# MrinalJain17/CT-image-segmentation

Hardware: AMD Instinct MI355X
Metric: CT volumes/sec training (512x512x48, bs=2/GPU) (higher is better)
Workload: dtype bf16; 1 GPU; 3D U-Net (MONAI UNet, channels 32-64-128-256, 2 res units) training step on 2x1x512x512x48 synthetic CT volumes per GPU (BASELINE.json configs[2]), CrossEntropy + Dice metric + Adam; global_batch=2, parallelism=dp1

## Files before the change

### ct-image-segmentation_amd/capstone_amd/_native.py

```python
import ctypes as C
import os

import torch

_HERE = os.path.dirname(os.path.abspath(__file__))
LIB_PATH = os.environ.get("CTSEG_LIB") or os.path.join(os.path.dirname(_HERE), "lib", "libctseg_hip.so")

F32, BF16, I16, U8, F16 = 0, 1, 2, 3, 4
MAX_TAPS, MAX_CLASSES = 27, 8
ABI_VERSION = 3
_TORCH_DT = {F32: torch.float32, BF16: torch.bfloat16, F16: torch.float16}
_EPC = {F32: 4, BF16: 8, F16: 8}
_SZ = {F32: 4, BF16: 2, F16: 2}
DT_OF_PRECISION = {"fp32": F32, "bf16": BF16, "fp16": F16}


def is16(dt):
    return dt in (BF16, F16)


def torch_dtype(dt):
    return _TORCH_DT[dt]


# ... 104 lines not shown
    "ctseg_instnorm_prelu_bwd_apply": (C.c_int, [_i32, _vp, _i32, _vp, _i32, _vp, _vp, _vp, _vp, _i32, _vp, _i32, _i32, _i64, _i32,
                                                 _vp, _i32, _vp, _vp]),
    "ctseg_instnorm_prelu_bwd_apply_colsum": (C.c_int, [_i32, _vp, _i32, _vp, _i32, _vp, _vp, _vp, _vp, _i32, _vp, _i32, _i32, _i64, _i32,
                                                        _vp, _i32, _vp, _vp, _i32, _vp, _vp]),
    "ctseg_colsum": (C.c_int, [_i32, _vp, _i32, _i64, _i32, _vp, _i32, _vp, _vp]),
    "ctseg_batchnorm_finalize": (C.c_int, [_vp, _i32, _i32, _i32, _i32, _i32, _f64, _f64, _f64, _vp, _vp, _vp, _vp, _vp, _vp, _vp, _vp]),
    "ctseg_batchnorm_eval_table": (C.c_int, [_vp, _vp, _vp, _vp, _i32, _f64, _vp, _vp]),
    "ctseg_scale_shift_prelu_fwd": (C.c_int, [_i32, _vp, _i32, _vp, _vp, _vp, _i32, _vp, _i32, _i32, _i64, _i32, _vp]),
    "ctseg_batchnorm_prelu_bwd_reduce": (C.c_int, [_i32, _vp, _i32, _vp, _i32, _vp, _vp, _vp, _vp, _vp, _i32, _i32, _i32, _i64, _i32,
                                                   _vp]),
    "ctseg_batchnorm_prelu_bwd_finalize": (C.c_int, [_vp, _i32, _i32, _i32, _i32, _f64, _vp, _vp, _vp, _vp, _vp]),
    "ctseg_batchnorm_prelu_bwd_apply": (C.c_int, [_i32, _vp, _i32, _vp, _i32, _vp, _vp, _vp, _vp, _vp, _vp, _i32, _vp, _i32, _i32,
                                                  _i64, _i32, _vp, _i32, _vp, _vp]),
    "ctseg_squash_masks": (C.c_int, [_vp, _i32, _i32, _i64, _vp, _vp, _vp, _vp]),
    "ctseg_squash_masks_present": (C.c_int, [_vp, _i32, _i32, _i64, _vp, _vp, _vp, _vp, _vp]),
    "ctseg_mixup_images": (C.c_int, [_vp, _vp, _i32, _i64, _f64, _vp, _vp]),
    "ctseg_seg_loss_pair": (C.c_int, [_vp, _i32, _vp, _vp, _i32, _i64, _i32, _vp, _i32, _vp, _i32, _vp, _vp, _vp, _i32, _i32, _vp]),
    "ctseg_seg_loss": (C.c_int, [_vp, _i32, _vp, _i32, _i64, _i32, _vp, _i32, _vp, _i32, _vp, _i32, _vp, _vp, _i32, _i32, _vp, _vp]),
    "ctseg_conv_logits_ce_slots": (C.c_int, [C.POINTER(ConvDesc), _i32]),
    "ctseg_conv_logits_ce": (C.c_int, [C.POINTER(ConvDesc), _vp, _i32, _vp, _vp, _i32, _vp, _i32, _vp, _i32, _i32, _vp, _vp]),
    "ctseg_dice_counts": (C.c_int, [_vp, _vp, _i32, _i64, _i32, _vp, _vp]),
    "ctseg_reduce_partials_f64": (C.c_int, [_vp, _i32, _i32, _i32, _vp, _vp]),
    "ctseg_loss_dice_summary": (C.c_int, [_vp, _i32, _i32, _vp, _i32, _vp, _vp]),
    "ctseg_adam_step": (C.c_int, [_vp, _vp, _vp, _vp, _i64, _f64, _f64, _f64, _f64, _i32, _f32, _vp]),
    "ctseg_scale_inplace": (C.c_int, [_vp, _i32, _i64, _vp, _f32, _vp]),
    "ctseg_cast": (C.c_int, [_vp, _i32, _vp, _i32, _i64, _vp]),
    "ctseg_nc_to_cl": (C.c_int, [_vp, _vp, _i32, _i32, _i32, _i64, _i32, _vp]),
    "ctseg_cl_to_nc": (C.c_int, [_vp, _i32, _vp, _i32, _i32, _i64, _i32, _vp]),
    "ctseg_resize3d_to_hwd": (C.c_int, [_vp, _i32, _vp] + [_i32] * 8 + [_f32, _f32, _vp, _vp, _vp, _vp, _vp]),
    "ctseg_window_gather": (C.c_int, [_vp] + [_i32] * 10 + [_f32, _vp, _i32, _i32, _vp]),
    "ctseg_window_gather_batch": (C.c_int, [_vp] + [_i32] * 4 + [_vp] + [_i32] * 4 + [_f32, _vp, _i32, _i32, _vp]),
    "ctseg_window_blend": (C.c_int, [_vp] + [_i32] * 8 + [_vp, _vp, _vp] + [_i32] * 4 + [_vp]),
    "ctseg_window_blend_batch": (C.c_int, [_vp] + [_i32] * 5 + [_vp, _i32, _vp, _vp, _vp] + [_i32] * 4 + [_vp, _vp]),
}
EXPORTS = tuple(_SIGS)
_lib = None


def lib():
    global _lib
    if _lib is None:
        if not os.path.exists(LIB_PATH):
            raise NativeError(f"{LIB_PATH} is missing: run `python -c 'import __graft_entry__ as g; g.build()'` "
                              "(or `make -C ct-image-segmentation_amd`). There is no CPU/eager fallback.")
        L = C.CDLL(LIB_PATH)
        for name, (res, args) in _SIGS.items():
            fn = getattr(L, name)
# ... 34 lines not shown
```

### ct-image-segmentation_amd/capstone_amd/engine.py

```python
import ctypes as C
import math
import os

import numpy as np
import torch

from . import _native as nat
from ._native import BF16, F32


def rup(a, b):
    return (a + b - 1) // b * b


class Act:
    __slots__ = ("t", "C", "c0", "dt", "pending_norm", "bst")

    def __init__(self, t, C, c0=0, dt=None):
        self.t, self.C, self.c0 = t, C, c0
        self.pending_norm = None
        self.bst = None
        self.dt = dt if dt is not None else {torch.float32: F32, torch.float16: nat.F16}.get(t.dtype, BF16)

    @property
# ... 135 lines not shown
    def g_ptr(self, p):
        return self.flat_g.data_ptr() + 4 * self.offsets[id(p)]

    def grad_view(self, p):
        o = self.offsets[id(p)]
        return self.flat_g[o:o + p.numel()].view(p.shape)

    def grad_views(self):
        if self._grad_views is None:
            self._grad_views = [self.grad_view(p) for p in self.params]
        return self._grad_views

    def version(self):
        return (self.generation, sum(p._version for p in self.params))

    def touch(self):
        self.generation += 1

    def ensure_adam_state(self):
        if self.adam_m is None:
            self.adam_m = torch.zeros_like(self.flat_g)
            self.adam_v = torch.zeros_like(self.flat_g)

    def adam_step(self, lr, betas=(0.9, 0.999), eps=1e-8, grad_scale=1.0):
        self.ensure_adam_state()
        self.step += 1
        nat.call("ctseg_adam_step", self.flat_p.data_ptr(), self.flat_g.data_ptr(), self.adam_m.data_ptr(),
                 self.adam_v.data_ptr(), self.n, lr, betas[0], betas[1], eps, self.step, grad_scale)
        self.touch()


class BufferStore:

    def __init__(self, norms, device):
        self.norms = list(norms)
        self.device = device
        self.offsets, off = {}, 0
        for i, m in enumerate(self.norms):
            self.offsets[id(m)] = (off, i)
            off += 2 * m.num_features
        self.flat = torch.zeros(max(off, 4), dtype=torch.float32, device=device)
        self.nbt = torch.zeros(max(len(self.norms), 1), dtype=torch.int64, device=device)
        self.copy_in()

    def _views(self, m):
        o, i = self.offsets[id(m)]
        C = m.num_features
        return self.flat[o:o + C], self.flat[o + C:o + 2 * C], self.nbt[i]

    def copy_in(self):
        with torch.no_grad():
            for m in self.norms:
# ... 323 lines not shown
                col0 += cout
        else:
            w, b, cout = self.parts[0]
            plan.emit("ctseg_conv_wgrad_reduce", ws.data_ptr(), nslabs, kpad_w, cn_pad, A, cg, self.T, 0, cn,
                      st.g_ptr(w), None)
            if b is not None and not bias_done:
                plan.emit_colsum(dy, st.g_ptr(b))


class NormStats:
    def __init__(self, plan, N, tiles, C, count):
        self.plan, self.N, self.tiles, self.C, self.count = plan, N, tiles, C, count
        self.ld = rup(C, 256 if C > 128 else nat.lib().ctseg_conv_tile_cols(C))
        self.partials = torch.zeros((N, tiles, 2, self.ld), dtype=torch.float32, device=plan.device)
        self.scratch = torch.zeros(N * 64 * 2 * self.ld + N, dtype=torch.float64, device=plan.device)

    def emit_finalize(self, col0, C, eps=1e-5):
        mr = torch.zeros((self.N, C, 2), dtype=torch.float32, device=self.plan.device)
        self.plan.emit("ctseg_instnorm_finalize", self.partials.data_ptr(), self.N, self.tiles, self.ld, col0, C,
                       float(self.count), float(eps), self.scratch.data_ptr(), mr.data_ptr(), keep=(self, mr))
        return mr


class Packer:
    def __init__(self, plan):
        self.plan = plan
        self.blocks = []
        self.descs = []
        self.total = 0
        self.bias_blocks, self.bias_total = [], 0
        self.first = (0, 0)
        self.buf = self.bias_buf = None
        self.idx = self.bias_idx = None
        self.n_idx = self.n_bidx = 0
        self.pack_blocks = self.pack_rows = None
        self.n_pack_blocks = self.n_pack_rows = 0
        self.n_first_rows = 0
        self.dirty = True
        self.version = None

    def add(self, layer, mode):
        dt = self.plan.dt
        bk = 128 // nat.elsize(dt)
        zero = self.plan.store.zero_index
        classes = layer.fwd_classes if mode == "fwd" else layer.dg_classes
        rows, gs = layer.rows_gather(mode)
        rows_pad = rup(rows, 256 if rows > 128 else 128)
        info = {"kpads": [], "w_offs": [], "base": self.total}
        for _, taps in classes:
            nt = len(taps)
            kpad = rup(nt * gs, bk)
            n_, t_, g_ = np.broadcast_arrays(np.arange(rows_pad)[:, None, None],
                                             np.array([t for t, _ in taps])[None, :, None],
                                             np.arange(gs)[None, None, :])
            src = np.where(n_ < rows, layer.src_index(mode, n_, g_, t_), zero)
            blk = np.full((rows_pad, kpad), zero, dtype=np.int64)
            blk[:, :nt * gs] = src.reshape(rows_pad, nt * gs)
            info["kpads"].append(kpad)
            info["w_offs"].append(self.total - info["base"])
            self.blocks.append((self.total, blk.reshape(-1)))
# ... 50 lines not shown
        self.dirty = True
        fits = all(sum((min(gh, d["gs"]) - gl) * d["T"] for (_, _, _, gl, gh, _, _) in d["parts"]) <= nat.PACK_LDS_FLOATS and
                   len(d["parts"]) <= 2 for d in self.descs)
        if self.descs and fits:
            arr = (nat.PackBlock * len(self.descs))()
            rows = []
            for b, d in enumerate(self.descs):
                B = arr[b]
                B.dst_off, B.kpad, B.gs, B.ntaps, B.T, B.nparts = d["dst_off"], d["kpad"], d["gs"], d["ntaps"], d["T"], len(d["parts"])
                for j, t in enumerate(d["taps"]):
                    B.tap[j] = t
                for k, (o, n_lo, n_hi, g_lo, g_hi, SN, SG) in enumerate(d["parts"]):
                    P = B.part[k]
                    P.o, P.n_lo, P.n_hi, P.g_lo, P.g_hi, P.SN, P.SG = o, n_lo, n_hi, g_lo, min(g_hi, d["gs"]), SN, SG
                rows += [(b, n) for n in range(d["rows"])]
            raw = torch.frombuffer(bytearray(bytes(arr)), dtype=torch.uint8).clone()
            self.pack_blocks = raw.to(dev)
            lo, hi = self.first
            head = [(b, n) for (b, n) in rows if lo <= self.descs[b]["dst_off"] < hi]
            rest = [(b, n) for (b, n) in rows if not (lo <= self.descs[b]["dst_off"] < hi)]
            self.n_first_rows = len(head)
            self.pack_rows = torch.tensor(head + rest, dtype=torch.int32).reshape(-1).to(dev)
            self.n_pack_blocks, self.n_pack_rows = len(self.descs), len(rows)

    def can_split(self):
        return self.pack_blocks is not None and self.n_first_rows > 0

    def stale(self):
        return self.dirty or self.plan.store.version() != self.version

    def refresh(self, force=False, part=None):
        st = self.plan.store
        ver = st.version()
        if not (force or self.dirty or ver != self.version):
            return
        if self.pack_blocks is not None:
            lo, hi = {None: (0, self.n_pack_rows), "first": (0, self.n_first_rows), "rest": (self.n_first_rows, self.n_pack_rows)}[part]
            if hi > lo:
                nat.call("ctseg_pack_weights", st.flat_p.data_ptr(), self.pack_blocks.data_ptr(), self.n_pack_blocks,
                         self.pack_rows.data_ptr() + 8 * lo, hi - lo, self.buf.data_ptr(), self.plan.dt)
        elif part != "rest":
            nat.call("ctseg_gather_cast", st.flat_p.data_ptr(), self.idx.data_ptr(), self.buf.data_ptr(), self.plan.dt, self.n_idx)
        if part != "rest":
            nat.call("ctseg_gather_cast", st.flat_p.data_ptr(), self.bias_idx.data_ptr(), self.bias_buf.data_ptr(), F32, self.n_bidx)
        if part != "first":
            self.dirty, self.version = False, ver
# ... 1 lines not shown
```

### ct-image-segmentation_amd/capstone_amd/plan.py

```python
import math
import os

import torch
import torch.nn as nn

from . import _native as nat
from ._native import BF16, F32
from .engine import Act, BufferStore, GemmLayer, NarrowUnsupported, Packer, ParamStore, plan_act, rup


def _is_seq(m):
    return isinstance(m, nn.Sequential) and not hasattr(m, "conv_only")


def _bwd_row_ranges(S, N, dt):
    P = max(1, min(1024, math.ceil(S / 512)))
    if nat.is16(dt):
        P = max(P, min(math.ceil(1024 / N), math.ceil(S / 32)))
    return P


def _parts(conv):
    return (conv.weight, conv.bias, conv.out_channels)

# ... 475 lines not shown
            return
        offs = [self.store.off(p) for p in params if p is not None]
        if self._pending_reduce:
            self._pending_ready.extend(offs)
            self._flush_reduces(only_if_chunk=True)
        else:
            self.ready_marks.append((len(self.bwd), offs))

    @staticmethod
    def run(prog, stream, lo=0, hi=None):
        for name, fn, args in prog[lo:hi]:
            rc = fn(*args, stream)
            if rc != 0:
                nat.check(rc, name)

    def load_input(self, x):
        N, X, Y, Z = self.shape
        cin = self.x.C
        xs = x.reshape(N, cin, X * Y * Z)
        if not xs.is_contiguous() or xs.dtype != torch.float32:
            xs = xs.contiguous().float()
        nat.call("ctseg_nc_to_cl", xs.data_ptr(), self.x.t.data_ptr(), self.dt, N, cin, X * Y * Z, cin)

    def repack_after_update(self):
        side = self.side_stream()
        if side is None:
            self.packer.dirty = True
            return
        main = torch.cuda.current_stream(self.device)
        side.wait_stream(main)
        with torch.cuda.stream(side):
            if self.packer.can_split():
                self.packer.refresh(force=True, part="first")
                self._repack_ev = side.record_event()
                self.packer.refresh(force=True, part="rest")
                self._repack_ev2 = side.record_event()
            else:
                self.packer.refresh(force=True)
                self._repack_ev = side.record_event()

    def head_ce_slots(self, n_classes):
        cache = self._head_ce
        if cache is None or cache[0] != n_classes:
            slots = 0
            name, _, args = self.fwd[-1]
            if name == "ctseg_conv_igemm" and not self.inference and args[0].out == self.logits.ptr():
                slots = nat.lib().ctseg_conv_logits_ce_slots(args[0], n_classes)
            cache = self._head_ce = (n_classes, max(slots, 0), args[0])
        return cache[1]

    def forward(self, x=None, skip_head=False):
        if x is not None:
            self.load_input(x)
        if self._repack_ev is not None:
            torch.cuda.current_stream(self.device).wait_event(self._repack_ev)
# ... 350 lines not shown
```

### ct-image-segmentation_amd/capstone_amd/segloss.py

```python
import contextlib
import math

import torch

from . import _native as nat
from ._native import BF16, F32

N_CLASSES = 10
CLASS_WEIGHT = (1e-10, 0.007, 0.3296, 0.0046, 0.2619, 0.3035, 0.0068, 0.0065, 0.0374, 0.0426)
SMOOTH = 1e-5
LOSS_NAMES = ("CrossEntropy", "WeightedCrossEntropy", "Focal", "Dice", "GeneralizedDice")


def cl_logits(t):
    if t.dtype != torch.float32 or not t.is_cuda or t.ndim < 3:
        return None
    perm = (0,) + tuple(range(2, t.ndim)) + (1,)
    v = t.permute(perm)
    st, sh = v.stride(), v.shape
    if st[-1] != 1:
        return None
    ld = st[-2] if v.ndim > 2 else sh[-1]
    exp = ld
    for d in range(v.ndim - 2, -1, -1):
# ... 52 lines not shown

    def set_labels_from_i64(self, target):
        t = target.reshape(self.B, self.S)
        self.labels = t.to(torch.uint8).contiguous()
        self.hist = torch.zeros((self.B, self.C), dtype=torch.int64, device=self.device)
        self.hist.scatter_add_(1, t.long(), torch.ones_like(t, dtype=torch.int64))

    def _pass(self, logits_ptr, ld, cw, do_stats, do_grad, coef=None, dl_ptr=None, g_ld=0, gdt=F32, pred=None, part=None):
        nat.call("ctseg_seg_loss", logits_ptr, ld, self.labels.data_ptr(), self.B, self.S, self.C, nat.ptr(cw),
                 int(do_stats), nat.ptr(part if part is not None else self.part), self.P, self.cnt.data_ptr(),
                 int(do_grad), nat.ptr(coef), dl_ptr, g_ld, gdt, nat.ptr(pred))

    def stats(self, logits_ptr, ld, weighted_too=False):
        self.cnt.zero_()
        self._pass(logits_ptr, ld, None, True, False)
        nat.call("ctseg_reduce_partials_f64", self.part.data_ptr(), self.B, self.P, self.R, self.red.data_ptr())
        if weighted_too:
            keep = self.cnt.clone()
            self._pass(logits_ptr, ld, self.cw, True, False)
            nat.call("ctseg_reduce_partials_f64", self.part.data_ptr(), self.B, self.P, self.R, self.red_w.data_ptr())
            self.cnt.copy_(keep)

    def prepare_fused_ce(self, weighted=False):
        self.cnt.zero_()
        w = self.cw.double() if weighted else torch.ones(self.C, dtype=torch.float64, device=self.device)
        denom = (self.hist.double() * w[None, :]).sum()
        self.coef.zero_()
        self.coef[:, 0] = (1.0 / denom).float()
        self._ce_ready = weighted

    def _take_ce_tables(self, weighted):
        if self._ce_ready is not weighted:
            self.prepare_fused_ce(weighted)
        self._ce_ready = None

    def fused_ce(self, logits_ptr, ld, dl_ptr, g_ld, gdt, weighted=False):
        self._take_ce_tables(weighted)
        self._pass(logits_ptr, ld, self.cw if weighted else None, 2, 2, self.coef, dl_ptr, g_ld, gdt)
        nat.call("ctseg_reduce_partials_f64", self.part.data_ptr(), self.B, self.P, self.R,
                 (self.red_w if weighted else self.red).data_ptr())

    def head_ce(self, desc, slots, dl_ptr, g_ld, weighted=False):
        self._take_ce_tables(weighted)
        part = self._part_head
        if part is None or part.shape[1] != slots:
            part = self._part_head = torch.zeros((self.B, slots, self.R), dtype=torch.float64, device=self.device)
        nat.call("ctseg_conv_logits_ce", desc, self.labels.data_ptr(), self.C, nat.ptr(self.cw if weighted else None),
                 self.coef.data_ptr(), self.coef.shape[1], dl_ptr, g_ld, part.data_ptr(), slots, self.R, self.cnt.data_ptr())
        nat.call("ctseg_reduce_partials_f64", part.data_ptr(), self.B, slots, self.R, (self.red_w if weighted else self.red).data_ptr())

    def ce_summary(self, weighted=False):
# ... 191 lines not shown
```

### ct-image-segmentation_amd/capstone_amd/volumetric/base_trainer.py

```python
from argparse import ArgumentParser
from typing import List

import torch
import torch.nn as nn

from .. import STRUCTURES, segloss
from .. import _native as nat
from ..models import UNet
from ..training.utils import _squash_predictions
from .losses import MultipleLossWrapper3D
from .metrics import DiceMetricWrapper3D
from .utils import _squash_masks_3D

try:
    import pytorch_lightning as pl
    _Base = pl.LightningModule
except Exception:
    pl = None

    class _HParams(dict):
        __getattr__ = dict.__getitem__

    class _Base(nn.Module):

# ... 271 lines not shown
            le.build_coef({n: 1.0 for n in names})
            le.grad(logits.ptr(), logits.ld, dl.ptr(), dl.ld, plan.dt)
        book = {}

        def bookkeeping():
            if ce_only:
                loss, dm, dpc = le.ce_summary(weighted=names[0] != "CrossEntropy")
                book["vals"], book["total"], book["dice"], book["packed"] = {names[0]: loss}, loss, (dm, dpc), le.last_summary
                return
            book["vals"] = vals
            book["total"] = torch.stack([vals[n] for n in names]).sum()
            book["dice"] = le.dice_metric()

        self._keep_dice_counts(le.cnt, "train")

        reducer = eng.reducer
        if reducer is not None:
            plan.backward(reducer.hooks(plan), before_join=bookkeeping)
            scale = reducer.finish()
        else:
            eng.warn_if_unattached()
            plan.backward(before_join=bookkeeping)
            scale = 1.0
        eng.store.adam_step(self.hparams.lr, betas, eps, grad_scale=scale)
        plan.repack_after_update()
        vals, total = book["vals"], book["total"]
        dice_mean, dice_per_class = book["dice"]
        if "packed" in book and pl is None:
            self.log_packed(book["packed"], [(f"{names[0]} Loss (train)", 0), ("Mean Dice Score (train)", 1),
                                             ("Dice per class (train)", slice(2, None))] +
                            [(f"{s_} Dice (train)", 2 + i) for i, s_ in enumerate(STRUCTURES)])
        else:
            for n in names:
                self.log(f"{n} Loss (train)", vals[n], on_step=False, on_epoch=True)
            self.log("Mean Dice Score (train)", dice_mean, on_step=False, on_epoch=True)
            if pl is None:
                self.log("Dice per class (train)", dice_per_class, on_step=False, on_epoch=True)
            else:
                for structure, score in zip(STRUCTURES, dice_per_class):
                    self.log(f"{structure} Dice (train)", score, on_step=False, on_epoch=True)
        return total

    def optimizer_state_dict(self, betas=(0.9, 0.999), eps=1e-8):
        st = self.unet.engine().store
        params = list(self.parameters())
        state = {}
        if st is not None and st.step > 0:
            for i, p in enumerate(params):
# ... 62 lines not shown
```

### ct-image-segmentation_amd/csrc/loss_metric.hip

```cpp
#include "loss_common.h"

namespace ctseg {

template <bool PRESENT>
__global__ __launch_bounds__(256) void squash_masks_kernel(const uint8_t* __restrict__ masks, int K, int64_t S,
                                                           uint8_t* __restrict__ labels, int64_t* __restrict__ labels_i64,
                                                           unsigned long long* __restrict__ hist, int* __restrict__ present) {
  __shared__ unsigned int s_h[32];
  __shared__ unsigned int s_pres;
  const int b = blockIdx.y;
  if (threadIdx.x < 32) s_h[threadIdx.x] = 0;
  if (PRESENT && threadIdx.x == 0) s_pres = 0u;
  unsigned int pres = 0u;
  __syncthreads();
  const uint8_t* mb = masks + (int64_t)b * K * S;
  int bg = 0;
  const bool vec = (S % 16 == 0) && (((uintptr_t)masks % 16) == 0) && (((uintptr_t)labels % 16) == 0);
  const int64_t nchunk = (S + 15) / 16;
  for (int64_t ch = blockIdx.x * (int64_t)blockDim.x + threadIdx.x; ch < nchunk; ch += (int64_t)gridDim.x * blockDim.x) {
    const int64_t v0 = ch * 16;
    int lab[16];
#pragma unroll
    for (int i = 0; i < 16; ++i) lab[i] = 0;
    if (vec) {
      for (int k = 0; k < K; ++k) {
        const u32x4 m = *reinterpret_cast<const u32x4*>(mb + (int64_t)k * S + v0);
        if constexpr (PRESENT) {
          unsigned int hit = 0u;
#pragma unroll
          for (int w = 0; w < 4; ++w) { const uint32_t z = m[w] ^ 0x01010101u; hit |= (z - 0x01010101u) & ~z & 0x80808080u; }
          if (hit) pres |= 1u << k;
        }
#pragma unroll
        for (int i = 0; i < 16; ++i) {
          const int val = (int)((m[i >> 2] >> (8 * (i & 3))) & 0xffu) * (k + 1);
          lab[i] = val > lab[i] ? val : lab[i];
        }
      }
      u32x4 o;
#pragma unroll
      for (int w = 0; w < 4; ++w)
        o[w] = (uint32_t)(lab[4 * w] & 0xff) | ((uint32_t)(lab[4 * w + 1] & 0xff) << 8) | ((uint32_t)(lab[4 * w + 2] & 0xff) << 16) |
               ((uint32_t)(lab[4 * w + 3] & 0xff) << 24);
      *reinterpret_cast<u32x4*>(labels + (int64_t)b * S + v0) = o;
    } else {
      for (int i = 0; i < 16; ++i) {
        if (v0 + i >= S) break;
        int l = 0;
        for (int k = 0; k < K; ++k) {
          const int mv = (int)mb[(int64_t)k * S + v0 + i];
          if (PRESENT && mv == 1) pres |= 1u << k;
          const int val = mv * (k + 1);
          l = val > l ? val : l;
        }
        lab[i] = l;
        labels[(int64_t)b * S + v0 + i] = (uint8_t)l;
      }
    }
    int nbg = 0;
#pragma unroll
    for (int i = 0; i < 16; ++i) {
      if (v0 + i < S) {
        if (labels_i64 != nullptr) labels_i64[(int64_t)b * S + v0 + i] = lab[i];
        if (lab[i] == 0) ++nbg;
        else if (lab[i] <= K) atomicAdd(&s_h[lab[i]], 1u);
      }
    }
    bg += nbg;
  }
#pragma unroll
  for (int o = 32; o > 0; o >>= 1) bg += __shfl_xor(bg, o, 64);
  if ((threadIdx.x & 63) == 0 && bg) atomicAdd(&s_h[0], (unsigned)bg);
  __syncthreads();
  if (threadIdx.x <= K && hist != nullptr && s_h[threadIdx.x] != 0)
    atomicAdd(&hist[(int64_t)b * (K + 1) + threadIdx.x], (unsigned long long)s_h[threadIdx.x]);
  if constexpr (PRESENT) {
#pragma unroll
    for (int o = 32; o > 0; o >>= 1) pres |= __shfl_xor(pres, o, 64);
    if ((threadIdx.x & 63) == 0 && pres) atomicOr(&s_pres, pres);
    __syncthreads();
    if (threadIdx.x < K && ((s_pres >> threadIdx.x) & 1u)) atomicOr(&present[(int64_t)b * K + threadIdx.x], 1);
  }
}

template <typename GT, bool SOFT, int CP>
__global__ __launch_bounds__(256) void seg_loss_kernel(const float* __restrict__ logits, int ld, const uint8_t* __restrict__ labels,
// ... 157 lines not shown
  if (t < C - 1) {
    const int c = t + 1;
    float sum = 0.f, n_ok = 0.f;
    for (int b = 0; b < B; ++b) {
      const float inter = (float)cnt[((int64_t)b * 3 + 0) * C + c], pred = (float)cnt[((int64_t)b * 3 + 1) * C + c],
                  truth = (float)cnt[((int64_t)b * 3 + 2) * C + c];
      if (truth > 0.f) { sum += 2.0f * inter / (truth + pred); n_ok += 1.f; }
    }
    const float pc = n_ok > 0.f ? sum / n_ok : 0.f;
    s_pc[t] = pc;
    out[2 + t] = pc;
  }
  __syncthreads();
  if (t == 0) {
    double a = 0.0, w = 0.0;
    for (int b = 0; b < B; ++b) { a += red[(int64_t)b * R]; w += red[(int64_t)b * R + 1]; }
    out[0] = (float)(a / w);
    float m = 0.f;
    for (int k = 0; k < C - 1; ++k) m += s_pc[k];
    out[1] = m / (float)(C - 1);
  }
}

}

using namespace ctseg;

extern "C" int ctseg_loss_dice_summary(const double* red, int32_t B, int32_t R, const int64_t* cnt, int32_t C, float* out,
                                       void* stream) {
  CTSEG_REQUIRE(red && cnt && out && B > 0 && R >= 2 && C >= 2 && C <= CMAX, "loss_dice_summary: bad arguments");
  hipLaunchKernelGGL(loss_dice_summary_kernel, dim3(1), dim3(64), 0, (hipStream_t)stream, red, B, R, (const long long*)cnt, C, out);
  CTSEG_LAUNCH_CHECK("loss_dice_summary");
  return 0;
}

static int squash_masks_launch(const uint8_t* masks, int32_t B, int32_t K, int64_t S, uint8_t* labels, int64_t* labels_i64,
                               int64_t* hist, int32_t* present, void* stream) {
  const int64_t nchunk = (S + 15) / 16;
  int64_t blocks = (nchunk + 255) / 256;
  if (blocks > 2048) blocks = 2048;
  if (present)
    hipLaunchKernelGGL(squash_masks_kernel<true>, dim3((unsigned)blocks, B), dim3(256), 0, (hipStream_t)stream, masks, K, S, labels,
                       labels_i64, (unsigned long long*)hist, present);
  else
    hipLaunchKernelGGL(squash_masks_kernel<false>, dim3((unsigned)blocks, B), dim3(256), 0, (hipStream_t)stream, masks, K, S, labels,
                       labels_i64, (unsigned long long*)hist, (int*)nullptr);
  return 0;
}

extern "C" int ctseg_squash_masks(const uint8_t* masks, int32_t B, int32_t K, int64_t S, uint8_t* labels, int64_t* labels_i64,
                                  int64_t* hist, void* stream) {
  CTSEG_REQUIRE(masks && labels && B > 0 && K > 0 && K < 32 && S > 0, "squash_masks: bad arguments");
  squash_masks_launch(masks, B, K, S, labels, labels_i64, hist, nullptr, stream);
  CTSEG_LAUNCH_CHECK("squash_masks");
  return 0;
}

extern "C" int ctseg_squash_masks_present(const uint8_t* masks, int32_t B, int32_t K, int64_t S, uint8_t* labels, int64_t* labels_i64,
                                          int64_t* hist, int32_t* present, void* stream) {
  CTSEG_REQUIRE(masks && labels && present && B > 0 && K > 0 && K < 32 && S > 0, "squash_masks_present: bad arguments");
  squash_masks_launch(masks, B, K, S, labels, labels_i64, hist, present, stream);
  CTSEG_LAUNCH_CHECK("squash_masks_present");
  return 0;
// ... 135 lines not shown
```

### ct-image-segmentation_amd/csrc/optim_misc.hip

```cpp
#include "ctseg_dev.h"

namespace ctseg {

static thread_local char g_err[512] = "";
void set_error(const char* fmt, ...) {
  va_list ap;
  va_start(ap, fmt);
  vsnprintf(g_err, sizeof(g_err), fmt, ap);
  va_end(ap);
}

__global__ __launch_bounds__(256) void adam_kernel(float* __restrict__ p, const float* __restrict__ g, float* __restrict__ m,
                                                   float* __restrict__ v, int64_t n, float omb1, float b2, float omb2, float eps,
                                                   float step_size, float bc2_sqrt, float gscale) {
  const int64_t n4 = n / 4;
  for (int64_t i = blockIdx.x * (int64_t)blockDim.x + threadIdx.x; i < n4; i += (int64_t)gridDim.x * blockDim.x) {
    f32x4 pp = reinterpret_cast<f32x4*>(p)[i], gg = reinterpret_cast<const f32x4*>(g)[i];
    f32x4 mm = reinterpret_cast<f32x4*>(m)[i], vv = reinterpret_cast<f32x4*>(v)[i];
#pragma unroll
    for (int e = 0; e < 4; ++e) {
      const float gr = gg[e] * gscale;
      mm[e] = mm[e] + (gr - mm[e]) * omb1;
      vv[e] = vv[e] * b2 + omb2 * gr * gr;
      const float denom = sqrtf(vv[e]) / bc2_sqrt + eps;
// ... 4 lines not shown
    reinterpret_cast<f32x4*>(v)[i] = vv;
  }
  if (blockIdx.x == 0 && threadIdx.x < (n & 3)) {
    const int64_t i = n4 * 4 + threadIdx.x;
    const float gr = g[i] * gscale;
    const float mm = m[i] + (gr - m[i]) * omb1;
    const float vv = v[i] * b2 + omb2 * gr * gr;
    m[i] = mm; v[i] = vv;
    p[i] = p[i] - step_size * (mm / (sqrtf(vv) / bc2_sqrt + eps));
  }
}

template <typename TD> __global__ void gather_cast_kernel(const float* __restrict__ src, const int32_t* __restrict__ idx,
                                                           TD* __restrict__ dst, int64_t n);
template <typename TS, typename TD> __device__ __forceinline__ TD cvt(TS x);
template <> __device__ __forceinline__ float cvt<float, float>(float x) { return x; }
template <> __device__ __forceinline__ unsigned short cvt<float, unsigned short>(float x) { return (unsigned short)f2bf(x); }
template <> __device__ __forceinline__ float cvt<unsigned short, float>(unsigned short x) { return bf2f(x); }
template <> __device__ __forceinline__ unsigned short cvt<unsigned short, unsigned short>(unsigned short x) { return x; }
template <> __device__ __forceinline__ _Float16 cvt<float, _Float16>(float x) {
  return __builtin_bit_cast(_Float16, (unsigned short)f2h<F16>(x));
}
template <> __device__ __forceinline__ float cvt<_Float16, float>(_Float16 x) { return (float)x; }

template <typename TD> __global__ void gather_cast_kernel(const float* __restrict__ src, const int32_t* __restrict__ idx,
                                                           TD* __restrict__ dst, int64_t n) {
  for (int64_t i = blockIdx.x * (int64_t)blockDim.x + threadIdx.x; i < n; i += (int64_t)gridDim.x * blockDim.x)
    dst[i] = cvt<float, TD>(src[idx[i]]);
}

template <typename TS, typename TD> __global__ void cast_kernel(const TS* __restrict__ s, TD* __restrict__ d, int64_t n) {
  for (int64_t i = blockIdx.x * (int64_t)blockDim.x + threadIdx.x; i < n; i += (int64_t)gridDim.x * blockDim.x)
    d[i] = cvt<TS, TD>(s[i]);
}

template <typename TD> __global__ __launch_bounds__(256) void pack_weights_kernel(const float* __restrict__ src,
                                                                                  const ctseg_pack_block* __restrict__ blocks,
                                                                                  const int32_t* __restrict__ rows, TD* __restrict__ dst) {
  __shared__ float s_w[CTSEG_PACK_LDS_FLOATS];
  const int b = rows[2 * blockIdx.x], n = rows[2 * blockIdx.x + 1];
  const ctseg_pack_block& B = blocks[b];
  const int T = B.T;
  int loff[2] = {0, 0};
#pragma unroll
  for (int p = 0; p < 2; ++p) {
    if (p < B.nparts) {
// ... 191 lines not shown

static inline unsigned nblocks(int64_t total, int cap = 4096) {
  int64_t b = (total + 255) / 256;
  return (unsigned)(b > cap ? cap : (b < 1 ? 1 : b));
}

}

using namespace ctseg;

extern "C" int ctseg_abi_version(void) { return CTSEG_ABI_VERSION; }
extern "C" const char* ctseg_last_error(void) { return g_err; }

extern "C" int ctseg_adam_step(float* p, const float* g, float* m, float* v, int64_t n, double lr, double beta1, double beta2,
                               double eps, int32_t step, float grad_scale, void* stream) {
  CTSEG_REQUIRE(p && g && m && v && n > 0 && step >= 1, "adam_step: bad arguments");
  CTSEG_REQUIRE(((uintptr_t)p % 16) == 0 && ((uintptr_t)g % 16) == 0 && ((uintptr_t)m % 16) == 0 && ((uintptr_t)v % 16) == 0,
                "adam_step: buffers must be 16-byte aligned");
  const double bc1 = 1.0 - pow(beta1, (double)step), bc2 = 1.0 - pow(beta2, (double)step);
  const float step_size = (float)(lr / bc1), bc2_sqrt = (float)sqrt(bc2);
  hipLaunchKernelGGL(adam_kernel, dim3(nblocks(n / 4 + 1, 2048)), dim3(256), 0, (hipStream_t)stream, p, g, m, v, n, (float)(1.0 - beta1),
                     (float)beta2, (float)(1.0 - beta2), (float)eps, step_size, bc2_sqrt, grad_scale);
  CTSEG_LAUNCH_CHECK("adam_step");
  return 0;
}

template <typename T> __global__ __launch_bounds__(256) void scale_inplace_kernel(T* __restrict__ x, int64_t n, const float* __restrict__ dev_scale,
                                                                                    float host_scale) {
  const float f = host_scale * (dev_scale ? *dev_scale : 1.f);
  if (f == 1.f) return;
  constexpr int V = 16 / sizeof(T);
  const int64_t nv = n / V;
  for (int64_t i = blockIdx.x * (int64_t)blockDim.x + threadIdx.x; i < nv; i += (int64_t)gridDim.x * blockDim.x) {
    if constexpr (sizeof(T) == 4) {
      f32x4 v = reinterpret_cast<f32x4*>(x)[i];
#pragma unroll
      for (int e = 0; e < 4; ++e) v[e] *= f;
      reinterpret_cast<f32x4*>(x)[i] = v;
    } else {
      u32x4 v = reinterpret_cast<u32x4*>(x)[i];
#pragma unroll
      for (int e = 0; e < 4; ++e) {
        const unsigned lo = (unsigned)f2bf(bf2f(v[e] & 0xffffu) * f), hi = (unsigned)f2bf(bf2f(v[e] >> 16) * f);
        v[e] = (lo & 0xffffu) | (hi << 16);
      }
      reinterpret_cast<u32x4*>(x)[i] = v;
// ... 173 lines not shown
```

### include/ctseg_hip.h

```cpp
#ifndef CTSEG_HIP_H
#define CTSEG_HIP_H

#include <stdint.h>

#ifdef __cplusplus
extern "C" {
#endif

#define CTSEG_ABI_VERSION 3
#define CTSEG_F32 0
#define CTSEG_BF16 1
#define CTSEG_I16 2
#define CTSEG_U8 3
#define CTSEG_F16 4
#define CTSEG_MAX_TAPS 27
#define CTSEG_MAX_CLASSES 8

int ctseg_abi_version(void);
const char* ctseg_last_error(void);

typedef struct ctseg_conv_class {
  int32_t ntaps;
  int32_t kpad;
  int64_t w_off;
// ... 151 lines not shown
                                    const float* sums, void* dy, int32_t dy_ld, void* g_copy, int32_t g_copy_ld, int32_t N,
                                    int64_t S, int32_t C, const double* da_part, int32_t n_da, float* dalpha, void* stream);

int ctseg_squash_masks(const uint8_t* masks, int32_t B, int32_t K, int64_t S, uint8_t* labels, int64_t* labels_i64,
                       int64_t* hist, void* stream);
int ctseg_squash_masks_present(const uint8_t* masks, int32_t B, int32_t K, int64_t S, uint8_t* labels, int64_t* labels_i64,
                               int64_t* hist, int32_t* present, void* stream);
int ctseg_mixup_images(const float* x, const int32_t* perm, int32_t B, int64_t n, double lambda, float* out, void* stream);

int ctseg_seg_loss(const float* logits, int32_t ld, const uint8_t* labels, int32_t B, int64_t S, int32_t C,
                   const float* class_weight, int32_t do_stats, double* part, int32_t P, int64_t* cnt, int32_t do_grad,
                   const float* coef, void* dlogits, int32_t g_ld, int32_t gdtype, uint8_t* pred_out, void* stream);
int ctseg_seg_loss_pair(const float* logits, int32_t ld, const uint8_t* labels, const int32_t* perm, int32_t B, int64_t S,
                        int32_t C, const float* class_weight, int32_t do_grad, double* part, int32_t P, int64_t* cnt,
                        const float* coef, void* dlogits, int32_t g_ld, int32_t gdtype, void* stream);
int ctseg_conv_logits_ce_slots(const ctseg_conv_desc* d, int32_t C);
int ctseg_conv_logits_ce(const ctseg_conv_desc* d, const uint8_t* labels, int32_t C, const float* class_weight, const float* coef,
                         int32_t coef_stride, void* dlogits, int32_t g_ld, double* part, int32_t P, int32_t R, int64_t* cnt,
                         void* stream);
int ctseg_dice_counts(const uint8_t* pred, const uint8_t* truth, int32_t B, int64_t S, int32_t C, int64_t* cnt, void* stream);
int ctseg_reduce_partials_f64(const double* part, int32_t B, int32_t P, int32_t R, double* out, void* stream);
int ctseg_loss_dice_summary(const double* red, int32_t B, int32_t R, const int64_t* cnt, int32_t C, float* out, void* stream);

int ctseg_adam_step(float* p, const float* g, float* m, float* v, int64_t n, double lr, double beta1, double beta2, double eps,
                    int32_t step, float grad_scale, void* stream);

int ctseg_scale_inplace(void* x, int32_t dtype, int64_t n, const float* dev_scale, float host_scale, void* stream);

int ctseg_cast(const void* src, int32_t src_dtype, void* dst, int32_t dst_dtype, int64_t n, void* stream);
int ctseg_nc_to_cl(const float* src, void* dst, int32_t dtype, int32_t N, int32_t C, int64_t S, int32_t ld, void* stream);
int ctseg_cl_to_nc(const void* src, int32_t dtype, float* dst, int32_t N, int32_t C, int64_t S, int32_t ld, void* stream);

int ctseg_resize3d_to_hwd(const void* image, int32_t image_dtype, const uint8_t* masks, int32_t K, int32_t D, int32_t H, int32_t W,
                          int32_t Do, int32_t Ho, int32_t Wo, int32_t window, float win_lo, float win_hi, float* image_out,
                          uint8_t* masks_out, uint8_t* labels_out, int64_t* hist, void* stream);

int ctseg_window_gather(const float* vol, int32_t Cin, int32_t X, int32_t Y, int32_t Z, int32_t x0, int32_t y0, int32_t z0,
                        int32_t rx, int32_t ry, int32_t rz, float cval, void* dst, int32_t dtype, int32_t ld, void* stream);
int ctseg_window_gather_batch(const float* vol, int32_t Cin, int32_t X, int32_t Y, int32_t Z, const int32_t* starts, int32_t nw,
                              int32_t rx, int32_t ry, int32_t rz, float cval, void* dst, int32_t dtype, int32_t ld, void* stream);
int ctseg_window_blend(const float* logits, int32_t ld, int32_t C, int32_t rx, int32_t ry, int32_t rz, int32_t x0, int32_t y0,
                       int32_t z0, const float* importance, const float* inv_count, float* out, int32_t X, int32_t Y, int32_t Z,
                       int32_t out_ld, void* stream);
int ctseg_window_blend_batch(const float* logits, int32_t ld, int32_t C, int32_t rx, int32_t ry, int32_t rz, const int32_t* starts,
                             int32_t nw, const float* importance, const float* inv_count, float* out, int32_t X, int32_t Y,
                             int32_t Z, int32_t out_ld, const int32_t* bbox, void* stream);

#ifdef __cplusplus
// ... 4 lines not shown
```

Before: 225.2 volumes/s.

## Fuse Adam with weight repacking, move CE prep to GPU, speed up mask squashing

```diff
diff --git a/ct-image-segmentation_amd/capstone_amd/_native.py b/ct-image-segmentation_amd/capstone_amd/_native.py
--- a/ct-image-segmentation_amd/capstone_amd/_native.py
+++ b/ct-image-segmentation_amd/capstone_amd/_native.py
@@ -150,7 +150,9 @@
     "ctseg_dice_counts": (C.c_int, [_vp, _vp, _i32, _i64, _i32, _vp, _vp]),
     "ctseg_reduce_partials_f64": (C.c_int, [_vp, _i32, _i32, _i32, _vp, _vp]),
     "ctseg_loss_dice_summary": (C.c_int, [_vp, _i32, _i32, _vp, _i32, _vp, _vp]),
+    "ctseg_ce_prepare": (C.c_int, [_vp, _i32, _i32, _vp, _vp, _i32, _vp, _vp]),
     "ctseg_adam_step": (C.c_int, [_vp, _vp, _vp, _vp, _i64, _f64, _f64, _f64, _f64, _i32, _f32, _vp]),
+    "ctseg_adam_step_packed": (C.c_int, [_vp, _vp, _vp, _vp, _i64, _f64, _f64, _f64, _f64, _i32, _f32, _vp, _vp, _vp, _i32, _vp, _vp]),
     "ctseg_scale_inplace": (C.c_int, [_vp, _i32, _i64, _vp, _f32, _vp]),
     "ctseg_cast": (C.c_int, [_vp, _i32, _vp, _i32, _i64, _vp]),
     "ctseg_nc_to_cl": (C.c_int, [_vp, _vp, _i32, _i32, _i32, _i64, _i32, _vp]),
diff --git a/ct-image-segmentation_amd/capstone_amd/engine.py b/ct-image-segmentation_amd/capstone_amd/engine.py
--- a/ct-image-segmentation_amd/capstone_amd/engine.py
+++ b/ct-image-segmentation_amd/capstone_amd/engine.py
@@ -181,12 +181,19 @@
             self.adam_m = torch.zeros_like(self.flat_g)
             self.adam_v = torch.zeros_like(self.flat_g)
 
-    def adam_step(self, lr, betas=(0.9, 0.999), eps=1e-8, grad_scale=1.0):
+    def adam_step(self, lr, betas=(0.9, 0.999), eps=1e-8, grad_scale=1.0, packer=None):
         self.ensure_adam_state()
         self.step += 1
-        nat.call("ctseg_adam_step", self.flat_p.data_ptr(), self.flat_g.data_ptr(), self.adam_m.data_ptr(),
-                 self.adam_v.data_ptr(), self.n, lr, betas[0], betas[1], eps, self.step, grad_scale)
+        sc = packer.scatter if packer is not None and packer.plan.store is self else None
+        if sc is not None:
+            nat.call("ctseg_adam_step_packed", self.flat_p.data_ptr(), self.flat_g.data_ptr(), self.adam_m.data_ptr(),
+                     self.adam_v.data_ptr(), self.n, lr, betas[0], betas[1], eps, self.step, grad_scale, sc["goff"].data_ptr(),
+                     sc["ent"].data_ptr(), packer.buf.data_ptr(), packer.plan.dt, packer.bias_buf.data_ptr())
+        else:
+            nat.call("ctseg_adam_step", self.flat_p.data_ptr(), self.flat_g.data_ptr(), self.adam_m.data_ptr(),
+                     self.adam_v.data_ptr(), self.n, lr, betas[0], betas[1], eps, self.step, grad_scale)
         self.touch()
+        return sc["part"] if sc is not None else None
 
 
 class BufferStore:
@@ -556,6 +563,44 @@
         return mr
 
 
+def build_scatter(n, zero_index, idx, ranges, bias_idx):
+    idx, bias_idx = np.asarray(idx, dtype=np.int64), np.asarray(bias_idx, dtype=np.int64)
+    dst, flag = [], []
+    for lo, hi in ranges:
+        d = np.arange(lo, hi, dtype=np.int64)
+        dst.append(d[idx[lo:hi] != zero_index])
+        flag.append(np.zeros(len(dst[-1]), dtype=np.int64))
+    d = np.arange(len(bias_idx), dtype=np.int64)
+    dst.append(d[bias_idx != zero_index])
+    flag.append(np.ones(len(dst[-1]), dtype=np.int64))
+    dst, flag = np.concatenate(dst), np.concatenate(flag)
+    src = np.where(flag == 1, bias_idx[np.minimum(dst, len(bias_idx) - 1)], idx[np.minimum(dst, len(idx) - 1)])
+    if len(dst) == 0 or dst.max() >= 1 << 29 or len(dst) >= 1 << 31 or src.min() < 0 or src.max() >= n:
+        return None
+    order = np.argsort(src, kind="stable")
+    src, dst, flag = src[order], dst[order], flag[order]
+    ng = n // 4 + 1
+    counts = np.bincount(src >> 2, minlength=ng)
+    goff = np.zeros(ng + 1, dtype=np.int64)
+    goff[1:] = np.cumsum(counts)
+    ent = (dst | ((src & 3) << 29) | (flag << 31)).astype(np.uint32)
+    grp = np.repeat(np.arange(ng, dtype=np.int64), counts)
+    e64 = ent.astype(np.int64)
+    back_src, back_dst, back_bias = 4 * grp + ((e64 >> 29) & 3), e64 & ((1 << 29) - 1), (e64 >> 31) == 1
+    assert np.array_equal(np.where(back_bias, bias_idx[np.minimum(back_dst, len(bias_idx) - 1)],
+                                   idx[np.minimum(back_dst, len(idx) - 1)]), back_src), "scatter table disagrees with the index"
+    seen = np.zeros(len(idx), dtype=np.int64)
+    np.add.at(seen, back_dst[~back_bias], 1)
+    want = np.zeros(len(idx), dtype=np.int64)
+    for lo, hi in ranges:
+        want[lo:hi] = idx[lo:hi] != zero_index
+    assert np.array_equal(seen, want), "scatter table does not cover the operand buffer exactly once"
+    seen_b = np.zeros(len(bias_idx), dtype=np.int64)
+    np.add.at(seen_b, back_dst[back_bias], 1)
+    assert np.array_equal(seen_b, (bias_idx != zero_index).astype(np.int64)), "scatter table does not cover the biases exactly once"
+    return goff.astype(np.int32), ent, int(np.bincount(src).max())
+
+
 class Packer:
     def __init__(self, plan):
         self.plan = plan
@@ -570,6 +615,7 @@
         self.pack_blocks = self.pack_rows = None
         self.n_pack_blocks = self.n_pack_rows = 0
         self.n_first_rows = 0
+        self.scatter = None
         self.dirty = True
         self.version = None
 
@@ -666,6 +712,27 @@
             self.n_first_rows = len(head)
             self.pack_rows = torch.tensor(head + rest, dtype=torch.int32).reshape(-1).to(dev)
             self.n_pack_blocks, self.n_pack_rows = len(self.descs), len(rows)
+        self._build_scatter(idx, bidx)
+
+    def _build_scatter(self, idx, bidx):
+        mode = os.environ.get("CTSEG_ADAM_PACKED", "first")
+        self.scatter = None
+        if mode == "0" or not nat.is16(self.plan.dt) or self.plan.device.type != "cuda" or self.total == 0:
+            return
+        if mode == "all":
+            part, ranges = "all", [(0, self.total)]
+        elif self.can_split():
+            part, ranges = "first", [self.first]
+        else:
+            return
+        st = self.plan.store
+        tab = build_scatter(st.n, st.zero_index, idx[:self.total], ranges, bidx)
+        if tab is None:
+            return
+        goff, ent, fan = tab
+        dev = self.plan.device
+        self.scatter = {"goff": torch.from_numpy(goff).to(dev), "ent": torch.from_numpy(ent.view(np.int32)).to(dev), "part": part,
+                        "fanout": fan}
 
     def can_split(self):
         return self.pack_blocks is not None and self.n_first_rows > 0
diff --git a/ct-image-segmentation_amd/capstone_amd/plan.py b/ct-image-segmentation_amd/capstone_amd/plan.py
--- a/ct-image-segmentation_amd/capstone_amd/plan.py
+++ b/ct-image-segmentation_amd/capstone_amd/plan.py
@@ -521,7 +521,10 @@
             xs = xs.contiguous().float()
         nat.call("ctseg_nc_to_cl", xs.data_ptr(), self.x.t.data_ptr(), self.dt, N, cin, X * Y * Z, cin)
 
-    def repack_after_update(self):
+    def repack_after_update(self, done=None):
+        if done == "all":
+            self.packer.dirty, self.packer.version = False, self.store.version()
+            return
         side = self.side_stream()
         if side is None:
             self.packer.dirty = True
@@ -529,7 +532,10 @@
         main = torch.cuda.current_stream(self.device)
         side.wait_stream(main)
         with torch.cuda.stream(side):
-            if self.packer.can_split():
+            if done == "first":
+                self.packer.refresh(force=True, part="rest")
+                self._repack_ev2 = side.record_event()
+            elif self.packer.can_split():
                 self.packer.refresh(force=True, part="first")
                 self._repack_ev = side.record_event()
                 self.packer.refresh(force=True, part="rest")
diff --git a/ct-image-segmentation_amd/capstone_amd/segloss.py b/ct-image-segmentation_amd/capstone_amd/segloss.py
--- a/ct-image-segmentation_amd/capstone_amd/segloss.py
+++ b/ct-image-segmentation_amd/capstone_amd/segloss.py
@@ -98,11 +98,19 @@
             self.cnt.copy_(keep)
 
     def prepare_fused_ce(self, weighted=False):
-        self.cnt.zero_()
-        w = self.cw.double() if weighted else torch.ones(self.C, dtype=torch.float64, device=self.device)
-        denom = (self.hist.double() * w[None, :]).sum()
-        self.coef.zero_()
-        self.coef[:, 0] = (1.0 / denom).float()
+        if torch.device(self.device).type != "cuda":
+            self.cnt.zero_()
+            w = self.cw.double() if weighted else torch.ones(self.C, dtype=torch.float64, device=self.device)
+            denom = (self.hist.double() * w[None, :]).sum()
+            self.coef.zero_()
+            self.coef[:, 0] = (1.0 / denom).float()
+            self._ce_ready = weighted
+            return
+        hist = self.hist
+        if hist.dtype != torch.int64 or not hist.is_contiguous():
+            hist = self.hist = hist.long().contiguous()
+        nat.call("ctseg_ce_prepare", hist.data_ptr(), self.B, self.C, nat.ptr(self.cw if weighted else None), self.coef.data_ptr(),
+                 self.coef.shape[1], self.cnt.data_ptr())
         self._ce_ready = weighted
 
     def _take_ce_tables(self, weighted):
diff --git a/ct-image-segmentation_amd/capstone_amd/volumetric/base_trainer.py b/ct-image-segmentation_amd/capstone_amd/volumetric/base_trainer.py
--- a/ct-image-segmentation_amd/capstone_amd/volumetric/base_trainer.py
+++ b/ct-image-segmentation_amd/capstone_amd/volumetric/base_trainer.py
@@ -317,8 +317,7 @@
             eng.warn_if_unattached()
             plan.backward(before_join=bookkeeping)
             scale = 1.0
-        eng.store.adam_step(self.hparams.lr, betas, eps, grad_scale=scale)
-        plan.repack_after_update()
+        plan.repack_after_update(eng.store.adam_step(self.hparams.lr, betas, eps, grad_scale=scale, packer=plan.packer))
         vals, total = book["vals"], book["total"]
         dice_mean, dice_per_class = book["dice"]
         if "packed" in book and pl is None:
diff --git a/ct-image-segmentation_amd/csrc/loss_metric.hip b/ct-image-segmentation_amd/csrc/loss_metric.hip
--- a/ct-image-segmentation_amd/csrc/loss_metric.hip
+++ b/ct-image-segmentation_amd/csrc/loss_metric.hip
@@ -2,6 +2,7 @@
 
 namespace ctseg {
 
+constexpr int SQ_PLANES = 9;
 template <bool PRESENT>
 __global__ __launch_bounds__(256) void squash_masks_kernel(const uint8_t* __restrict__ masks, int K, int64_t S,
                                                            uint8_t* __restrict__ labels, int64_t* __restrict__ labels_i64,
@@ -16,34 +17,84 @@
   const uint8_t* mb = masks + (int64_t)b * K * S;
   int bg = 0;
   const bool vec = (S % 16 == 0) && (((uintptr_t)masks % 16) == 0) && (((uintptr_t)labels % 16) == 0);
+  const bool vec64 = ((uintptr_t)labels_i64 % 16) == 0;
   const int64_t nchunk = (S + 15) / 16;
   for (int64_t ch = blockIdx.x * (int64_t)blockDim.x + threadIdx.x; ch < nchunk; ch += (int64_t)gridDim.x * blockDim.x) {
     const int64_t v0 = ch * 16;
     int lab[16];
-#pragma unroll
-    for (int i = 0; i < 16; ++i) lab[i] = 0;
     if (vec) {
-      for (int k = 0; k < K; ++k) {
-        const u32x4 m = *reinterpret_cast<const u32x4*>(mb + (int64_t)k * S + v0);
-        if constexpr (PRESENT) {
-          unsigned int hit = 0u;
-#pragma unroll
-          for (int w = 0; w < 4; ++w) { const uint32_t z = m[w] ^ 0x01010101u; hit |= (z - 0x01010101u) & ~z & 0x80808080u; }
-          if (hit) pres |= 1u << k;
-        }
-#pragma unroll
-        for (int i = 0; i < 16; ++i) {
-          const int val = (int)((m[i >> 2] >> (8 * (i & 3))) & 0xffu) * (k + 1);
-          lab[i] = val > lab[i] ? val : lab[i];
-        }
-      }
-      u32x4 o;
-#pragma unroll
-      for (int w = 0; w < 4; ++w)
-        o[w] = (uint32_t)(lab[4 * w] & 0xff) | ((uint32_t)(lab[4 * w + 1] & 0xff) << 8) | ((uint32_t)(lab[4 * w + 2] & 0xff) << 16) |
-               ((uint32_t)(lab[4 * w + 3] & 0xff) << 24);
-      *reinterpret_cast<u32x4*>(labels + (int64_t)b * S + v0) = o;
+      u32x4 lw = {0u, 0u, 0u, 0u};
+      bool bytewise = false;
+      for (int k0 = 0; k0 < K; k0 += SQ_PLANES) {
+        u32x4 m[SQ_PLANES];
+#pragma unroll
+        for (int j = 0; j < SQ_PLANES; ++j) {
+          const int k = k0 + j < K ? k0 + j : K - 1;
+          m[j] = *reinterpret_cast<const u32x4*>(mb + (int64_t)k * S + v0);
+        }
+        uint32_t other = 0u;
+#pragma unroll
+        for (int j = 0; j < SQ_PLANES; ++j)
+          if (k0 + j < K) other |= (m[j][0] | m[j][1] | m[j][2] | m[j][3]) & 0xfefefefeu;
+        if (other != 0u && !bytewise) {
+          bytewise = true;
+#pragma unroll
+          for (int i = 0; i < 16; ++i) lab[i] = (int)((lw[i >> 2] >> (8 * (i & 3))) & 0xffu);
+        }
+#pragma unroll
+        for (int j = 0; j < SQ_PLANES; ++j) {
+          if (k0 + j < K) {
+            const int k = k0 + j;
+            if constexpr (PRESENT) {
+              unsigned int hit = 0u;
+#pragma unroll
+              for (int w = 0; w < 4; ++w) { const uint32_t z = m[j][w] ^ 0x01010101u; hit |= (z - 0x01010101u) & ~z & 0x80808080u; }
+              if (hit) pres |= 1u << k;
+            }
+            if (!bytewise) {
+#pragma unroll
+              for (int w = 0; w < 4; ++w) {
+                const uint32_t sel = m[j][w] * 0xffu;
+                lw[w] = (lw[w] & ~sel) | (m[j][w] * (uint32_t)(k + 1));
+              }
+            } else {
+#pragma unroll
+              for (int i = 0; i < 16; ++i) {
+                const int val = (int)((m[j][i >> 2] >> (8 * (i & 3))) & 0xffu) * (k + 1);
+                lab[i] = val > lab[i] ? val : lab[i];
+              }
+            }
+          }
+        }
+      }
+      if (bytewise) {
+#pragma unroll
+        for (int w = 0; w < 4; ++w)
+          lw[w] = (uint32_t)(lab[4 * w] & 0xff) | ((uint32_t)(lab[4 * w + 1] & 0xff) << 8) | ((uint32_t)(lab[4 * w + 2] & 0xff) << 16) |
+                  ((uint32_t)(lab[4 * w + 3] & 0xff) << 24);
+      }
+      *reinterpret_cast<u32x4*>(labels + (int64_t)b * S + v0) = lw;
+      if (!bytewise) {
+        if ((lw[0] | lw[1] | lw[2] | lw[3]) == 0u) {
+          bg += 16;
+          if (labels_i64 != nullptr) {
+            int64_t* l64 = labels_i64 + (int64_t)b * S + v0;
+            if (vec64) {
+#pragma unroll
+              for (int i = 0; i < 8; ++i) reinterpret_cast<u32x4*>(l64)[i] = u32x4{0u, 0u, 0u, 0u};
+            } else {
+#pragma unroll
+              for (int i = 0; i < 16; ++i) l64[i] = 0;
+            }
+          }
+          continue;
+        }
+#pragma unroll
+        for (int i = 0; i < 16; ++i) lab[i] = (int)((lw[i >> 2] >> (8 * (i & 3))) & 0xffu);
+      }
     } else {
+#pragma unroll
+      for (int i = 0; i < 16; ++i) lab[i] = 0;
       for (int i = 0; i < 16; ++i) {
         if (v0 + i >= S) break;
         int l = 0;
@@ -58,10 +109,20 @@
       }
     }
     int nbg = 0;
+    if (labels_i64 != nullptr) {
+      int64_t* l64 = labels_i64 + (int64_t)b * S + v0;
+      if (vec && vec64) {
+#pragma unroll
+        for (int i = 0; i < 8; ++i) reinterpret_cast<u32x4*>(l64)[i] = u32x4{(uint32_t)lab[2 * i], 0u, (uint32_t)lab[2 * i + 1], 0u};
+      } else {
+#pragma unroll
+        for (int i = 0; i < 16; ++i)
+          if (v0 + i < S) l64[i] = lab[i];
+      }
+    }
 #pragma unroll
     for (int i = 0; i < 16; ++i) {
       if (v0 + i < S) {
-        if (labels_i64 != nullptr) labels_i64[(int64_t)b * S + v0 + i] = lab[i];
         if (lab[i] == 0) ++nbg;
         else if (lab[i] <= K) atomicAdd(&s_h[lab[i]], 1u);
       }
@@ -265,6 +326,17 @@
   }
 }
 
+__global__ __launch_bounds__(64) void ce_prepare_kernel(const long long* __restrict__ hist, int B, int C, const float* __restrict__ cw,
+                                                         float* __restrict__ coef, int ncoef, long long* __restrict__ cnt) {
+  const int t = threadIdx.x;
+  for (int i = t; i < B * 3 * C; i += 64) cnt[i] = 0;
+  double denom = 0.0;
+  for (int b = 0; b < B; ++b)
+    for (int c = 0; c < C; ++c) denom += (double)hist[(int64_t)b * C + c] * (cw ? (double)cw[c] : 1.0);
+  const float inv = (float)(1.0 / denom);
+  for (int i = t; i < B * ncoef; i += 64) coef[i] = (i % ncoef) == 0 ? inv : 0.f;
+}
+
 }
 
 using namespace ctseg;
@@ -277,11 +349,20 @@
   return 0;
 }
 
+extern "C" int ctseg_ce_prepare(const int64_t* hist, int32_t B, int32_t C, const float* class_weight, float* coef, int32_t ncoef,
+                                int64_t* cnt, void* stream) {
+  CTSEG_REQUIRE(hist && coef && cnt && B > 0 && C >= 2 && C <= CMAX && ncoef >= 1, "ce_prepare: bad arguments");
+  hipLaunchKernelGGL(ce_prepare_kernel, dim3(1), dim3(64), 0, (hipStream_t)stream, (const long long*)hist, B, C, class_weight, coef,
+                     ncoef, (long long*)cnt);
+  CTSEG_LAUNCH_CHECK("ce_prepare");
+  return 0;
+}
+
 static int squash_masks_launch(const uint8_t* masks, int32_t B, int32_t K, int64_t S, uint8_t* labels, int64_t* labels_i64,
                                int64_t* hist, int32_t* present, void* stream) {
   const int64_t nchunk = (S + 15) / 16;
   int64_t blocks = (nchunk + 255) / 256;
-  if (blocks > 2048) blocks = 2048;
+  if (blocks > 16384) blocks = 16384;
   if (present)
     hipLaunchKernelGGL(squash_masks_kernel<true>, dim3((unsigned)blocks, B), dim3(256), 0, (hipStream_t)stream, masks, K, S, labels,
                        labels_i64, (unsigned long long*)hist, present);
diff --git a/ct-image-segmentation_amd/csrc/optim_misc.hip b/ct-image-segmentation_amd/csrc/optim_misc.hip
--- a/ct-image-segmentation_amd/csrc/optim_misc.hip
+++ b/ct-image-segmentation_amd/csrc/optim_misc.hip
@@ -50,6 +50,57 @@
   return __builtin_bit_cast(_Float16, (unsigned short)f2h<F16>(x));
 }
 template <> __device__ __forceinline__ float cvt<_Float16, float>(_Float16 x) { return (float)x; }
+
+template <typename TD>
+__global__ __launch_bounds__(256) void adam_packed_kernel(float* __restrict__ p, const float* __restrict__ g, float* __restrict__ m,
+                                                          float* __restrict__ v, int64_t n, float omb1, float b2, float omb2, float eps,
+                                                          float step_size, float bc2_sqrt, float gscale,
+                                                          const int32_t* __restrict__ goff, const uint32_t* __restrict__ ent,
+                                                          TD* __restrict__ buf, float* __restrict__ bias_buf) {
+  const int64_t n4 = n / 4;
+  for (int64_t i = blockIdx.x * (int64_t)blockDim.x + threadIdx.x; i < n4; i += (int64_t)gridDim.x * blockDim.x) {
+    f32x4 pp = reinterpret_cast<f32x4*>(p)[i], gg = reinterpret_cast<const f32x4*>(g)[i];
+    f32x4 mm = reinterpret_cast<f32x4*>(m)[i], vv = reinterpret_cast<f32x4*>(v)[i];
+    const int j0 = goff[i], j1 = goff[i + 1];
+#pragma unroll
+    for (int e = 0; e < 4; ++e) {
+      const float gr = gg[e] * gscale;
+      mm[e] = mm[e] + (gr - mm[e]) * omb1;
+      vv[e] = vv[e] * b2 + omb2 * gr * gr;
+      const float denom = sqrtf(vv[e]) / bc2_sqrt + eps;
+      pp[e] = pp[e] - step_size * (mm[e] / denom);
+    }
+    reinterpret_cast<f32x4*>(p)[i] = pp;
+    reinterpret_cast<f32x4*>(m)[i] = mm;
+    reinterpret_cast<f32x4*>(v)[i] = vv;
+    for (int j = j0; j < j1; ++j) {
+      const uint32_t en = ent[j], lane = (en >> 29) & 3u, d = en & 0x1fffffffu;
+      const float x = lane == 0 ? pp[0] : lane == 1 ? pp[1] : lane == 2 ? pp[2] : pp[3];
+      if (en >> 31) bias_buf[d] = x;
+      else buf[d] = cvt<float, TD>(x);
+    }
+  }
+  if (blockIdx.x == 0 && threadIdx.x < (n & 3)) {
+    const int64_t i = n4 * 4 + threadIdx.x;
+    const float gr = g[i] * gscale;
+    const float mm = m[i] + (gr - m[i]) * omb1;
+    float vv;
+    {
+#pragma clang fp contract(off)
+      const float a = v[i] * b2, b = omb2 * gr * gr;
+      vv = a + b;
+    }
+    m[i] = mm; v[i] = vv;
+    const float x = p[i] - step_size * (mm / (sqrtf(vv) / bc2_sqrt + eps));
+    p[i] = x;
+    for (int j = goff[n4]; j < goff[n4 + 1]; ++j) {
+      const uint32_t en = ent[j], d = en & 0x1fffffffu;
+      if (((en >> 29) & 3u) != threadIdx.x) continue;
+      if (en >> 31) bias_buf[d] = x;
+      else buf[d] = cvt<float, TD>(x);
+    }
+  }
+}
 
 template <typename TD> __global__ void gather_cast_kernel(const float* __restrict__ src, const int32_t* __restrict__ idx,
                                                            TD* __restrict__ dst, int64_t n) {
@@ -287,6 +338,27 @@
   hipLaunchKernelGGL(adam_kernel, dim3(nblocks(n / 4 + 1, 2048)), dim3(256), 0, (hipStream_t)stream, p, g, m, v, n, (float)(1.0 - beta1),
                      (float)beta2, (float)(1.0 - beta2), (float)eps, step_size, bc2_sqrt, grad_scale);
   CTSEG_LAUNCH_CHECK("adam_step");
+  return 0;
+}
+
+extern "C" int ctseg_adam_step_packed(float* p, const float* g, float* m, float* v, int64_t n, double lr, double beta1, double beta2,
+                                      double eps, int32_t step, float grad_scale, const int32_t* group_off, const uint32_t* entries,
+                                      void* buf, int32_t dtype, float* bias_buf, void* stream) {
+  CTSEG_REQUIRE(p && g && m && v && n > 0 && step >= 1 && group_off && entries && buf && bias_buf, "adam_step_packed: bad arguments");
+  CTSEG_REQUIRE(is16(dtype), "adam_step_packed: 16-bit operand storage only (fp32 storage: ctseg_adam_step, then the packers)");
+  CTSEG_REQUIRE(((uintptr_t)p % 16) == 0 && ((uintptr_t)g % 16) == 0 && ((uintptr_t)m % 16) == 0 && ((uintptr_t)v % 16) == 0,
+                "adam_step_packed: buffers must be 16-byte aligned");
+  const double bc1 = 1.0 - pow(beta1, (double)step), bc2 = 1.0 - pow(beta2, (double)step);
+  const float step_size = (float)(lr / bc1), bc2_sqrt = (float)sqrt(bc2);
+  const dim3 grid(nblocks(n / 4 + 1, 2048)), blk(256);
+  if (dtype == CTSEG_F16)
+    hipLaunchKernelGGL(adam_packed_kernel<_Float16>, grid, blk, 0, (hipStream_t)stream, p, g, m, v, n, (float)(1.0 - beta1), (float)beta2,
+                       (float)(1.0 - beta2), (float)eps, step_size, bc2_sqrt, grad_scale, group_off, entries, (_Float16*)buf, bias_buf);
+  else
+    hipLaunchKernelGGL(adam_packed_kernel<unsigned short>, grid, blk, 0, (hipStream_t)stream, p, g, m, v, n, (float)(1.0 - beta1),
+                       (float)beta2, (float)(1.0 - beta2), (float)eps, step_size, bc2_sqrt, grad_scale, group_off, entries,
+                       (unsigned short*)buf, bias_buf);
+  CTSEG_LAUNCH_CHECK("adam_step_packed");
   return 0;
 }
 
diff --git a/include/ctseg_hip.h b/include/ctseg_hip.h
--- a/include/ctseg_hip.h
+++ b/include/ctseg_hip.h
@@ -197,8 +197,15 @@
 int ctseg_reduce_partials_f64(const double* part, int32_t B, int32_t P, int32_t R, double* out, void* stream);
 int ctseg_loss_dice_summary(const double* red, int32_t B, int32_t R, const int64_t* cnt, int32_t C, float* out, void* stream);
 
+int ctseg_ce_prepare(const int64_t* hist, int32_t B, int32_t C, const float* class_weight, float* coef, int32_t ncoef, int64_t* cnt,
+                     void* stream);
+
 int ctseg_adam_step(float* p, const float* g, float* m, float* v, int64_t n, double lr, double beta1, double beta2, double eps,
                     int32_t step, float grad_scale, void* stream);
+
+int ctseg_adam_step_packed(float* p, const float* g, float* m, float* v, int64_t n, double lr, double beta1, double beta2, double eps,
+                           int32_t step, float grad_scale, const int32_t* group_off, const uint32_t* entries, void* buf, int32_t dtype,
+                           float* bias_buf, void* stream);
 
 int ctseg_scale_inplace(void* x, int32_t dtype, int64_t n, const float* dev_scale, float host_scale, void* stream);
 
```

After: 224.6 volumes/s. No clear change (-0.3%).
